# LouisPwr/CarpeDeam

Hardware: AMD Instinct MI355X
Metric: corrected bases/sec on 50M×100bp synthetic reads (dhigh), 1/2/4/8 GPU (higher is better)
Workload: dtype u8 (2-bit packed bases; int32 scores; software x87 f80 likelihood sums)

## Files before the change

carpedeam_amd/csrc/rescore.hip:

```cpp
#include "scan.h"

#include <cfloat>
#include <climits>

#include "common.h"
#include "devutil.h"

namespace {

struct RescoreArgs {
    MetaWoff woff; MetaLen len; MetaHasN hasN; MetaRaw hasRaw;
    const uint32_t *codes, *nmask; const uint8_t *raw;
    const uint64_t *hoff;
    const HitRec *hit;
    const int32_t *minScore;
    uint64_t nHits;
    uint32_t n;
    float seqIdThr, covThr;
    int covMode, minAlnLen;
    AlnRec *tmp;
    uint16_t *tmpRy;
    uint8_t *valid;
    unsigned int *undef;
};

__device__ __forceinline__ bool canBeCovered(float covThr, int covMode, float ql, float tl) {
    switch (covMode) {
        case 0: return ((ql / tl >= covThr) && (tl / ql >= covThr));
        case 2: return ((tl / ql) >= covThr);
        case 1: return ((ql / tl) >= covThr);
        case 3: return ((tl / ql) >= covThr) && (tl / ql) <= 1.0;
        case 4: return ((ql / tl) >= covThr) && (ql / tl) <= 1.0;
        case 5: return (fminf(tl, ql) / fmaxf(tl, ql)) >= covThr;
        default: return true;
    }
}
__device__ __forceinline__ bool hasCoverage(float covThr, int covMode, float qc, float tc) {
    switch (covMode) { case 0: return qc >= covThr && tc >= covThr; case 2: return qc >= covThr; case 1: return tc >= covThr; default: return true; }
}
__device__ __forceinline__ float computeCov(unsigned s, unsigned e, unsigned len) {
    return (min(len, max(s, e)) - min(s, e) + 1) / (float) len;
}

__device__ __forceinline__ void orientedBase(const RescoreArgs &a, uint32_t w0, uint32_t L, bool hasN, bool rc, uint32_t i, uint32_t &code, bool &isN) {
    const uint32_t p = rc ? (L - 1 - i) : i;
    code = cdm_base(a.codes, w0, p);
    isN = hasN && cdm_isN(a.nmask, w0, p);
    if (rc) code = 3u - code;
}

struct Diag { unsigned score; unsigned diagLen; unsigned dist; int diagonal; unsigned ident; unsigned ry; bool any; unsigned first, last; };

__device__ __forceinline__ void scoreDiagonal(const RescoreArgs &a, uint32_t qw, uint32_t qLen, bool qN, bool rc, uint32_t tw, uint32_t tLen, bool tN,
                                              int diagonal, Diag &best, bool qRaw = false, bool tRaw = false) {
    const unsigned md = (unsigned) abs(diagonal);
    uint32_t qOff, tOff, m;
    if (diagonal >= 0 && md < qLen) { qOff = md; tOff = 0; m = min(tLen, qLen - md); }
    else if (diagonal < 0 && md < tLen) { qOff = 0; tOff = md; m = min(tLen - md, qLen); }
    else return;
    unsigned mism = 0, identN = 0, ry = 0xFFFFu;
    uint32_t first = 0, last = m - 1;
    if (qRaw || tRaw) {
        const uint8_t q0 = (qRaw && !rc) ? cdm_raw_at(a.raw, qw, qOff) : 0, t0 = tRaw ? cdm_raw_at(a.raw, tw, tOff) : 0;
        const uint8_t q1 = (qRaw && !rc) ? cdm_raw_at(a.raw, qw, qOff + m - 1) : 0, t1 = tRaw ? cdm_raw_at(a.raw, tw, tOff + m - 1) : 0;
        first = (q0 == '*' || t0 == '*') ? 1u : 0u;
        if (last > 0 && (q1 == '*' || t1 == '*')) last--;
    }
    if (!qN && !tN) {
        ry = 0;
        const uint32_t qLast = (qLen + 15) / 16 - 1, tLast = (tLen + 15) / 16 - 1;
        for (uint32_t k = 0; k < m; k += 16) {
            const uint32_t x = cdm_oriented_window16(a.codes, qw, qLen, qLast, rc, qOff + k) ^ cdm_window16(a.codes, tw, tOff + k, tLast);
            uint32_t mm = (x | (x >> 1)) & 0x55555555u;
            const uint32_t rem = m - k;
            uint32_t rr = x & 0x55555555u;
            if (rem < 16) { mm &= (1u << (2 * rem)) - 1u; rr &= (1u << (2 * rem)) - 1u; }
            mism += __popc(mm); ry += __popc(rr);
        }
    } else {
        for (uint32_t k = first; k <= last && k < m; k++) {
            uint32_t qc, tc; bool qn, tn;
            orientedBase(a, qw, qLen, qN, rc, qOff + k, qc, qn);
            orientedBase(a, tw, tLen, tN, false, tOff + k, tc, tn);
            const bool match = !qn && !tn && qc == tc;
            mism += !match;
            if (!qRaw && !tRaw) identN += (qn && tn && !rc);
            else {
                uint8_t ql = qn ? (rc ? 'X' : 'N') : (uint8_t) "ACGT"[qc], tl = tn ? 'N' : (uint8_t) "ACGT"[tc];
                if (qRaw && !rc) ql = cdm_raw_at(a.raw, qw, qOff + k);
                if (tRaw) tl = cdm_raw_at(a.raw, tw, tOff + k);
                identN += ((ql & 0xDFu) == (tl & 0xDFu)) - (int) match;
            }
        }
    }
    const uint32_t cols = last + 1u >= first ? last + 1u - first : 0u;
    const long long sc = 2ll * (cols - mism) - 3ll * mism;
    const unsigned score = sc > 0 ? (unsigned) sc : 0u;
    if (score > best.score) { best.score = score; best.diagLen = m; best.dist = md; best.diagonal = diagonal; best.ident = (cols - mism) + identN; best.ry = ry; best.any = true; best.first = first; best.last = last; }
}

__global__ __launch_bounds__(256) void k_rescore(RescoreArgs a, const uint32_t *__restrict__ hitQuery) {
    const uint64_t h = (uint64_t) blockIdx.x * blockDim.x + threadIdx.x;
    if (h >= a.nHits) return;
    const uint32_t q = hitQuery[h];
    const HitRec hit = a.hit[h];
    const uint32_t t = hit.target;
    const uint32_t qLen = a.len[q], tLen = a.len[t], qw = a.woff[q], tw = a.woff[t];
    const bool qN = a.hasN[q] != 0, tN = a.hasN[t] != 0;
    const bool qRaw = qN && a.hasRaw[q] != 0, tRaw = tN && a.hasRaw[t] != 0;
    const bool isReverse = hit.score < 0;
    const bool isIdentity = (q == t);
    a.valid[h] = 0;
    if (!canBeCovered(a.covThr, a.covMode, (float) qLen, (float) tLen)) return;
    const unsigned short u = (unsigned short) (short) hit.diagonal;
    Diag best; best.score = 0; best.diagLen = 0; best.dist = 0; best.diagonal = 0; best.ident = 0; best.ry = 0xFFFFu; best.any = false; best.first = 0; best.last = 0;
    for (unsigned d = 1; d <= 1 + tLen / 32768; d++) scoreDiagonal(a, qw, qLen, qN, isReverse, tw, tLen, tN, (int) (-(int) d * 65536 + (int) u), best, qRaw, tRaw);
    for (unsigned d = 0; d <= qLen / 65536; d++) scoreDiagonal(a, qw, qLen, qN, isReverse, tw, tLen, tN, (int) (d * 65536 + u), best, qRaw, tRaw);
    if (!best.any) {
        if (!isIdentity) return;
        AlnRec r; r.target = t; r.rawScore = 0; r.ident = 1; r.qStart = r.qEnd = r.dbStart = r.dbEnd = -1; r.seqId = 1.0f;
        a.tmp[h] = r; a.tmpRy[h] = 0xFFFFu; a.valid[h] = 1;
        atomicAdd(a.undef, 1u);
        return;
    }
    const int startPos = (int) best.first, endPos = (int) best.last;
    const int alnLen = (endPos - startPos) + 1;
    int qs, qe, ds, de;
    if (best.diagonal >= 0) { qs = startPos + (int) best.dist; qe = endPos + (int) best.dist; ds = startPos; de = endPos; }
    else { qs = startPos; qe = endPos; ds = startPos + (int) best.dist; de = endPos + (int) best.dist; }
    const bool hasEvalue = (int) best.score >= a.minScore[qLen];
    float seqId = 0.f;
    if (hasEvalue || isIdentity) seqId = static_cast<float>(best.ident) / static_cast<float>(alnLen);
    const float queryCov = computeCov(qs, qe, qLen), targetCov = computeCov(ds, de, tLen);
    if (isReverse) { qs = (int) qLen - qs - 1; qe = (int) qLen - qe - 1; }
    const bool hasCov = hasCoverage(a.covThr, a.covMode, queryCov, targetCov);
    const bool hasSeqId = (double) seqId >= (double) (a.seqIdThr - FLT_EPSILON);
    const bool hasAlnLen = alnLen >= a.minAlnLen;
    if (!(isIdentity || (hasAlnLen && hasCov && hasSeqId && hasEvalue))) return;
    AlnRec r;
    r.target = t; r.rawScore = (int) best.score; r.ident = (int) best.ident; r.qStart = qs; r.qEnd = qe; r.dbStart = ds; r.dbEnd = de;
    r.seqId = (seqId == 1.0f) ? 1.0f : (float) ((double) (int) (seqId * 1000) / 1000.0);
    a.tmp[h] = r;
    a.tmpRy[h] = (uint16_t) min(best.ry, 0xFFFFu);
    a.valid[h] = 1;
}

__global__ void k_expand(const uint64_t *__restrict__ off, uint32_t n, uint32_t *__restrict__ owner) {
    const uint32_t q = blockIdx.x * blockDim.x + threadIdx.x;
    if (q >= n) return;
    for (uint64_t h = off[q]; h < off[q + 1]; h++) owner[h] = q;
}
__global__ void k_count_valid(const uint64_t *__restrict__ off, const uint8_t *__restrict__ valid, uint32_t n, uint64_t *__restrict__ cnt) {
    const uint32_t q = blockIdx.x * blockDim.x + threadIdx.x;
    if (q >= n) return;
    uint64_t c = 0;
    for (uint64_t h = off[q]; h < off[q + 1]; h++) c += valid[h];
    cnt[q] = c;
}
constexpr uint32_t SCATTER_SMALL = 256;
__global__ void k_scatter(const uint64_t *__restrict__ off, const uint32_t *__restrict__ owner, const uint8_t *__restrict__ valid, const AlnRec *__restrict__ tmp,
                          const uint16_t *__restrict__ tmpRy, uint64_t nHits, const uint64_t *__restrict__ outOff, AlnRec *__restrict__ out, uint16_t *__restrict__ outRy) {
    const uint64_t h = (uint64_t) blockIdx.x * blockDim.x + threadIdx.x;
    if (h >= nHits || !valid[h]) return;
    const uint32_t q = owner[h];
    const uint64_t first = off[q];
    if (off[q + 1] - first > SCATTER_SMALL) return;
    uint64_t o = outOff[q];
    for (uint64_t j = first; j < h; j++) o += valid[j];
    out[o] = tmp[h]; outRy[o] = tmpRy[h];
}
__global__ void k_scatter_big(const uint64_t *__restrict__ off, const uint8_t *__restrict__ valid, const AlnRec *__restrict__ tmp, const uint16_t *__restrict__ tmpRy, uint32_t n,
                              const uint64_t *__restrict__ outOff, AlnRec *__restrict__ out, uint16_t *__restrict__ outRy) {
    const uint32_t q = blockIdx.x * blockDim.x + threadIdx.x;
    if (q >= n || off[q + 1] - off[q] <= SCATTER_SMALL) return;
    uint64_t o = outOff[q];
    for (uint64_t h = off[q]; h < off[q + 1]; h++) if (valid[h]) { out[o] = tmp[h]; outRy[o] = tmpRy[h]; o++; }
}
__global__ void k_len_hist(const uint32_t *__restrict__ len, uint32_t n, uint32_t *__restrict__ present) {
    const uint32_t i = blockIdx.x * blockDim.x + threadIdx.x;
    if (i < n) present[len[i]] = 1;
}

}

int cdm_rescore_impl(cdm_ctx *ctx, const cdm_seqdb *db, const cdm_hits *hits, const cdm_rescore_params *par, cdm_alns **out) {
    hipStream_t s = ctx->stream;
    const uint32_t n = (uint32_t) db->n;
    const uint64_t nHits = hits->count;
    if (db->maxLen >= (1u << 30)) { cdm_set_error("cdm_rescore: sequence too long"); return CDM_ERR_UNSUPPORTED; }
    if (nHits >= 0xFFFFFF00ull) { cdm_set_error("cdm_rescore: %llu prefilter hits (a call takes fewer than 2^32)", (unsigned long long) nHits); return CDM_ERR_UNSUPPORTED; }
    DevBuf<unsigned int> undef;
    if (!undef.alloc(2)) { cdm_set_error("cdm_rescore: out of device memory"); return CDM_ERR_HIP; }
    CDM_HIP(hipMemsetAsync(undef.p, 0, 8, s));
    DevBuf<uint32_t> dPresent, owner; DevBuf<int32_t> dMin; DevBuf<AlnRec> tmp; DevBuf<uint16_t> tmpRy; DevBuf<uint8_t> valid; DevBuf<uint64_t> cnt;
    if (!dPresent.alloc(db->maxLen + 1) || !dMin.alloc(db->maxLen + 1) || !owner.alloc(nHits) || !tmp.alloc(nHits) || !tmpRy.alloc(nHits) || !valid.alloc(nHits) || !cnt.alloc((size_t) n + 1)) {
        cdm_set_error("cdm_rescore: out of device memory"); return CDM_ERR_HIP;
    }
    std::vector<uint32_t> present(db->maxLen + 1);
    CDM_HIP(hipMemsetAsync(dPresent.p, 0, (size_t) (db->maxLen + 1) * 4, s));
    hipLaunchKernelGGL(k_len_hist, dim3((n + 255) / 256), dim3(256), 0, s, db->len, n, dPresent.p);
    CDM_HIP(hipMemcpyAsync(present.data(), dPresent.p, (size_t) (db->maxLen + 1) * 4, hipMemcpyDeviceToHost, s));
    CDM_HIP(hipStreamSynchronize(s));
    std::vector<int32_t> minScore(db->maxLen + 1, INT_MAX);
    for (uint32_t L = 1; L <= db->maxLen; L++) {
        if (!present[L]) continue;
        int lo = 0, hi = 2 * (int) L;
        if (!(cdm_evalue_host(hi, L, db->residues) <= par->eval_thr)) continue;
        while (lo < hi) { int mid = (lo + hi) / 2; if (cdm_evalue_host(mid, L, db->residues) <= par->eval_thr) hi = mid; else lo = mid + 1; }
        minScore[L] = lo;
    }
    CDM_HIP(hipMemcpyAsync(dMin.p, minScore.data(), (size_t) (db->maxLen + 1) * 4, hipMemcpyHostToDevice, s));
    hipLaunchKernelGGL(k_expand, dim3((n + 255) / 256), dim3(256), 0, s, hits->off, n, owner.p);
    DevBuf<SeqMeta> meta;
    MetaUniform uni;
    if (int rc = cdm_build_meta(ctx, db, &meta.p, &uni)) return rc;
    RescoreArgs a;
    cdmSetMeta(a, meta.p, uni); a.codes = db->codes; a.nmask = db->nmask; a.raw = db->raw; a.hoff = hits->off; a.hit = hits->rec;
    a.minScore = dMin.p; a.nHits = nHits; a.n = n; a.seqIdThr = par->seq_id_thr; a.covThr = par->cov_thr; a.covMode = par->cov_mode;
    a.minAlnLen = par->min_aln_len; a.tmp = tmp.p; a.tmpRy = tmpRy.p; a.valid = valid.p; a.undef = undef.p;
    hipEventRecord(ctx->ev0, s);
    if (nHits) hipLaunchKernelGGL(k_rescore, CDM_GRID((nHits + 255) / 256, 256), dim3(256), 0, s, a, owner.p);
    hipEventRecord(ctx->ev1, s);
    hipLaunchKernelGGL(k_count_valid, dim3((n + 255) / 256), dim3(256), 0, s, hits->off, valid.p, n, cnt.p);
    CDM_LAUNCH_CHECK();
    cdm_alns *res = new cdm_alns(); res->n = n;
    struct Guard { cdm_alns *&r; bool armed = true; ~Guard() { if (armed && r) { cdm_alns_free(r); r = nullptr; } } } guard{res};
    if (cdmMalloc(&res->off, ((size_t) n + 1) * 8) != hipSuccess) { cdm_set_error("cdm_rescore: out of device memory"); return CDM_ERR_HIP; }
    cdmscan::ScanTemp scanTmp;
    CDM_HIP(hipMemsetAsync(cnt.p + n, 0, 8, s));
    if (int rc = cdmscan::exclusiveScan<uint64_t>(s, scanTmp, cnt.p, res->off, (size_t) n + 1)) return rc;
    uint64_t total = 0; unsigned int nUndef = 0;
    CDM_HIP(hipMemcpyAsync(&total, res->off + n, 8, hipMemcpyDeviceToHost, s));
    CDM_HIP(hipMemcpyAsync(&nUndef, undef.p, 4, hipMemcpyDeviceToHost, s));
    { hipError_t e = hipStreamSynchronize(s); if (e != hipSuccess) { cdm_set_error("cdm_rescore: kernel failed: %s", hipGetErrorString(e)); return CDM_ERR_HIP; } }
    res->count = total; res->undefinedRecords = nUndef;
    if (cdmMalloc(&res->rec, (total + 1) * sizeof(AlnRec)) != hipSuccess || cdmMalloc(&res->ryMism, (total + 1) * sizeof(uint16_t)) != hipSuccess) { cdm_set_error("cdm_rescore: out of device memory"); return CDM_ERR_HIP; }
    res->rySerial = db->serial;
    if (nHits) hipLaunchKernelGGL(k_scatter, CDM_GRID((nHits + 255) / 256, 256), dim3(256), 0, s, hits->off, (const uint32_t *) owner.p, valid.p, tmp.p, tmpRy.p, (uint64_t) nHits, res->off, res->rec, res->ryMism);
    hipLaunchKernelGGL(k_scatter_big, dim3((n + 255) / 256), dim3(256), 0, s, hits->off, valid.p, tmp.p, tmpRy.p, n, res->off, res->rec, res->ryMism);
    { hipError_t e = hipStreamSynchronize(s); if (e != hipSuccess) { cdm_set_error("cdm_rescore: compaction failed: %s", hipGetErrorString(e)); return CDM_ERR_HIP; } }
    hipEventElapsedTime(&ctx->lastMs[1], ctx->ev0, ctx->ev1);
    guard.armed = false;
    *out = res;
    return CDM_OK;
}
```

Baseline: 17.40 billion.

## Fuse rescore output compaction into a single-pass decoupled look-back scan

Rescoring and output compaction now happen in one kernel. Each 256-hit tile takes a dynamic ticket, counts its valid alignments with a wave ballot, and gets its global offset through a decoupled look-back over per-tile status words. Records go straight to their final position, and per-query offsets are written from that. This drops the temporary record, ry and valid buffers, the count kernel, the exclusive scan, the two scatter kernels and one host sync. In exchange, the output arrays are sized for all hits rather than the exact total. Empty queries that fall past a bounded run need a fallback fill kernel, and the status memset covers one more element than is allocated.

After: 17.26 billion. No clear change (-0.8%).

```diff
diff --git a/carpedeam_amd/csrc/rescore.hip b/carpedeam_amd/csrc/rescore.hip
--- a/carpedeam_amd/csrc/rescore.hip
+++ b/carpedeam_amd/csrc/rescore.hip
@@ -1,4 +1,3 @@
-#include "scan.h"
 
 #include <cfloat>
 #include <climits>
@@ -18,10 +17,14 @@
     uint32_t n;
     float seqIdThr, covThr;
     int covMode, minAlnLen;
-    AlnRec *tmp;
-    uint16_t *tmpRy;
-    uint8_t *valid;
+    AlnRec *rec;
+    uint16_t *ry;
+    uint64_t *off;
+    unsigned long long *status;
+    unsigned long long *total;
+    unsigned int *ticket;
     unsigned int *undef;
+    unsigned int *longRun;
 };
 
 __device__ __forceinline__ bool canBeCovered(float covThr, int covMode, float ql, float tl) {
@@ -99,29 +102,24 @@
     if (score > best.score) { best.score = score; best.diagLen = m; best.dist = md; best.diagonal = diagonal; best.ident = (cols - mism) + identN; best.ry = ry; best.any = true; best.first = first; best.last = last; }
 }
 
-__global__ __launch_bounds__(256) void k_rescore(RescoreArgs a, const uint32_t *__restrict__ hitQuery) {
-    const uint64_t h = (uint64_t) blockIdx.x * blockDim.x + threadIdx.x;
-    if (h >= a.nHits) return;
-    const uint32_t q = hitQuery[h];
-    const HitRec hit = a.hit[h];
+__device__ __forceinline__ bool scoreHit(const RescoreArgs &a, uint32_t q, const HitRec hit, AlnRec &r, uint32_t &ry) {
     const uint32_t t = hit.target;
     const uint32_t qLen = a.len[q], tLen = a.len[t], qw = a.woff[q], tw = a.woff[t];
     const bool qN = a.hasN[q] != 0, tN = a.hasN[t] != 0;
     const bool qRaw = qN && a.hasRaw[q] != 0, tRaw = tN && a.hasRaw[t] != 0;
     const bool isReverse = hit.score < 0;
     const bool isIdentity = (q == t);
-    a.valid[h] = 0;
-    if (!canBeCovered(a.covThr, a.covMode, (float) qLen, (float) tLen)) return;
+    if (!canBeCovered(a.covThr, a.covMode, (float) qLen, (float) tLen)) return false;
     const unsigned short u = (unsigned short) (short) hit.diagonal;
     Diag best; best.score = 0; best.diagLen = 0; best.dist = 0; best.diagonal = 0; best.ident = 0; best.ry = 0xFFFFu; best.any = false; best.first = 0; best.last = 0;
     for (unsigned d = 1; d <= 1 + tLen / 32768; d++) scoreDiagonal(a, qw, qLen, qN, isReverse, tw, tLen, tN, (int) (-(int) d * 65536 + (int) u), best, qRaw, tRaw);
     for (unsigned d = 0; d <= qLen / 65536; d++) scoreDiagonal(a, qw, qLen, qN, isReverse, tw, tLen, tN, (int) (d * 65536 + u), best, qRaw, tRaw);
     if (!best.any) {
-        if (!isIdentity) return;
-        AlnRec r; r.target = t; r.rawScore = 0; r.ident = 1; r.qStart = r.qEnd = r.dbStart = r.dbEnd = -1; r.seqId = 1.0f;
-        a.tmp[h] = r; a.tmpRy[h] = 0xFFFFu; a.valid[h] = 1;
+        if (!isIdentity) return false;
+        r.target = t; r.rawScore = 0; r.ident = 1; r.qStart = r.qEnd = r.dbStart = r.dbEnd = -1; r.seqId = 1.0f;
+        ry = 0xFFFFu;
         atomicAdd(a.undef, 1u);
-        return;
+        return true;
     }
     const int startPos = (int) best.first, endPos = (int) best.last;
     const int alnLen = (endPos - startPos) + 1;
@@ -136,13 +134,72 @@
     const bool hasCov = hasCoverage(a.covThr, a.covMode, queryCov, targetCov);
     const bool hasSeqId = (double) seqId >= (double) (a.seqIdThr - FLT_EPSILON);
     const bool hasAlnLen = alnLen >= a.minAlnLen;
-    if (!(isIdentity || (hasAlnLen && hasCov && hasSeqId && hasEvalue))) return;
-    AlnRec r;
+    if (!(isIdentity || (hasAlnLen && hasCov && hasSeqId && hasEvalue))) return false;
     r.target = t; r.rawScore = (int) best.score; r.ident = (int) best.ident; r.qStart = qs; r.qEnd = qe; r.dbStart = ds; r.dbEnd = de;
     r.seqId = (seqId == 1.0f) ? 1.0f : (float) ((double) (int) (seqId * 1000) / 1000.0);
-    a.tmp[h] = r;
-    a.tmpRy[h] = (uint16_t) min(best.ry, 0xFFFFu);
-    a.valid[h] = 1;
+    ry = min(best.ry, 0xFFFFu);
+    return true;
+}
+
+constexpr int RS_TILE = 256, RS_WAVES = RS_TILE / 64;
+constexpr uint32_t RS_RUN = 32;
+constexpr unsigned long long ST_AGG = 1ull << 62, ST_PREFIX = 2ull << 62, ST_MASK = (1ull << 62) - 1ull;
+__global__ __launch_bounds__(RS_TILE) void k_rescore(RescoreArgs a, const uint32_t *__restrict__ hitQuery) {
+    __shared__ unsigned int sTile, sWave[RS_WAVES];
+    __shared__ unsigned long long sPrefix;
+    const int tid = threadIdx.x, lane = tid & 63, wave = tid >> 6;
+    if (tid == 0) sTile = atomicAdd(a.ticket, 1u);
+    __syncthreads();
+    const uint64_t tile = sTile, h = tile * RS_TILE + tid;
+    const bool live = h < a.nHits;
+    uint32_t q = 0, ry = 0xFFFFu;
+    AlnRec r;
+    bool ok = false;
+    if (live) { q = hitQuery[h]; ok = scoreHit(a, q, a.hit[h], r, ry); }
+    const unsigned long long m = __ballot(ok);
+    const uint32_t inWave = __builtin_amdgcn_mbcnt_hi((uint32_t) (m >> 32), __builtin_amdgcn_mbcnt_lo((uint32_t) m, 0u));
+    if (lane == 0) sWave[wave] = (uint32_t) __popcll(m);
+    __syncthreads();
+    uint32_t before = 0, tot = 0;
+#pragma unroll
+    for (int w = 0; w < RS_WAVES; w++) { const uint32_t c = sWave[w]; if (w < wave) before += c; tot += c; }
+    if (wave == 0) {
+        unsigned long long excl = 0;
+        if (tile == 0) { if (lane == 0) __hip_atomic_store(&a.status[0], ST_PREFIX | (unsigned long long) tot, __ATOMIC_RELAXED, __HIP_MEMORY_SCOPE_AGENT); }
+        else {
+            if (lane == 0) __hip_atomic_store(&a.status[tile], ST_AGG | (unsigned long long) tot, __ATOMIC_RELAXED, __HIP_MEMORY_SCOPE_AGENT);
+            long long t0 = (long long) tile - 1;
+            while (true) {
+                const long long t = t0 - lane;
+                unsigned long long v = ST_PREFIX;
+                if (t >= 0) do { v = __hip_atomic_load(&a.status[t], __ATOMIC_RELAXED, __HIP_MEMORY_SCOPE_AGENT); } while ((v >> 62) == 0ull);
+                const unsigned long long pm = __ballot((v >> 62) == 2ull);
+                const int first = pm ? __ffsll(pm) - 1 : 63;
+                const unsigned long long part = cdm_wave_incl_sum<unsigned long long>(lane <= first ? (v & ST_MASK) : 0ull);
+                excl += (unsigned long long) __shfl((long long) part, 63, 64);
+                if (pm) break;
+                t0 -= 64;
+            }
+            if (lane == 0) __hip_atomic_store(&a.status[tile], ST_PREFIX | (excl + tot), __ATOMIC_RELAXED, __HIP_MEMORY_SCOPE_AGENT);
+        }
+        if (lane == 0) sPrefix = excl;
+    }
+    __syncthreads();
+    if (!live) return;
+    const uint64_t o = sPrefix + before + inWave;
+    if (ok) { a.rec[o] = r; a.ry[o] = (uint16_t) ry; }
+    if (h == a.hoff[q]) {
+        a.off[q] = o;
+        uint32_t p = q;
+        while (p > 0 && q - p < RS_RUN && a.hoff[p - 1] == h) a.off[--p] = o;
+        if (p > 0 && a.hoff[p - 1] == h) *a.longRun = 1u;
+    }
+    if (h == a.nHits - 1) {
+        const uint64_t e = o + (ok ? 1u : 0u);
+        a.off[a.n] = e; *a.total = e;
+        if (a.n - 1 - q <= RS_RUN) for (uint32_t p = q + 1; p < a.n; p++) a.off[p] = e;
+        else *a.longRun = 1u;
+    }
 }
 
 __global__ void k_expand(const uint64_t *__restrict__ off, uint32_t n, uint32_t *__restrict__ owner) {
@@ -150,31 +207,11 @@
     if (q >= n) return;
     for (uint64_t h = off[q]; h < off[q + 1]; h++) owner[h] = q;
 }
-__global__ void k_count_valid(const uint64_t *__restrict__ off, const uint8_t *__restrict__ valid, uint32_t n, uint64_t *__restrict__ cnt) {
+__global__ void k_fill_empty(const uint64_t *__restrict__ hoff, const uint32_t *__restrict__ owner, uint32_t n, uint64_t nHits, uint64_t total, uint64_t *off) {
     const uint32_t q = blockIdx.x * blockDim.x + threadIdx.x;
     if (q >= n) return;
-    uint64_t c = 0;
-    for (uint64_t h = off[q]; h < off[q + 1]; h++) c += valid[h];
-    cnt[q] = c;
-}
-constexpr uint32_t SCATTER_SMALL = 256;
-__global__ void k_scatter(const uint64_t *__restrict__ off, const uint32_t *__restrict__ owner, const uint8_t *__restrict__ valid, const AlnRec *__restrict__ tmp,
-                          const uint16_t *__restrict__ tmpRy, uint64_t nHits, const uint64_t *__restrict__ outOff, AlnRec *__restrict__ out, uint16_t *__restrict__ outRy) {
-    const uint64_t h = (uint64_t) blockIdx.x * blockDim.x + threadIdx.x;
-    if (h >= nHits || !valid[h]) return;
-    const uint32_t q = owner[h];
-    const uint64_t first = off[q];
-    if (off[q + 1] - first > SCATTER_SMALL) return;
-    uint64_t o = outOff[q];
-    for (uint64_t j = first; j < h; j++) o += valid[j];
-    out[o] = tmp[h]; outRy[o] = tmpRy[h];
-}
-__global__ void k_scatter_big(const uint64_t *__restrict__ off, const uint8_t *__restrict__ valid, const AlnRec *__restrict__ tmp, const uint16_t *__restrict__ tmpRy, uint32_t n,
-                              const uint64_t *__restrict__ outOff, AlnRec *__restrict__ out, uint16_t *__restrict__ outRy) {
-    const uint32_t q = blockIdx.x * blockDim.x + threadIdx.x;
-    if (q >= n || off[q + 1] - off[q] <= SCATTER_SMALL) return;
-    uint64_t o = outOff[q];
-    for (uint64_t h = off[q]; h < off[q + 1]; h++) if (valid[h]) { out[o] = tmp[h]; outRy[o] = tmpRy[h]; o++; }
+    const uint64_t h = hoff[q];
+    if (h == hoff[q + 1]) off[q] = h < nHits ? off[owner[h]] : total;
 }
 __global__ void k_len_hist(const uint32_t *__restrict__ len, uint32_t n, uint32_t *__restrict__ present) {
     const uint32_t i = blockIdx.x * blockDim.x + threadIdx.x;
@@ -189,13 +226,14 @@
     const uint64_t nHits = hits->count;
     if (db->maxLen >= (1u << 30)) { cdm_set_error("cdm_rescore: sequence too long"); return CDM_ERR_UNSUPPORTED; }
     if (nHits >= 0xFFFFFF00ull) { cdm_set_error("cdm_rescore: %llu prefilter hits (a call takes fewer than 2^32)", (unsigned long long) nHits); return CDM_ERR_UNSUPPORTED; }
-    DevBuf<unsigned int> undef;
-    if (!undef.alloc(2)) { cdm_set_error("cdm_rescore: out of device memory"); return CDM_ERR_HIP; }
-    CDM_HIP(hipMemsetAsync(undef.p, 0, 8, s));
-    DevBuf<uint32_t> dPresent, owner; DevBuf<int32_t> dMin; DevBuf<AlnRec> tmp; DevBuf<uint16_t> tmpRy; DevBuf<uint8_t> valid; DevBuf<uint64_t> cnt;
-    if (!dPresent.alloc(db->maxLen + 1) || !dMin.alloc(db->maxLen + 1) || !owner.alloc(nHits) || !tmp.alloc(nHits) || !tmpRy.alloc(nHits) || !valid.alloc(nHits) || !cnt.alloc((size_t) n + 1)) {
+    const uint64_t tiles = (nHits + RS_TILE - 1) / RS_TILE;
+    DevBuf<unsigned long long> ctl, status;
+    DevBuf<uint32_t> dPresent, owner; DevBuf<int32_t> dMin;
+    if (!ctl.alloc(3) || !status.alloc(tiles) || !dPresent.alloc(db->maxLen + 1) || !dMin.alloc(db->maxLen + 1) || !owner.alloc(nHits)) {
         cdm_set_error("cdm_rescore: out of device memory"); return CDM_ERR_HIP;
     }
+    CDM_HIP(hipMemsetAsync(ctl.p, 0, 24, s));
+    CDM_HIP(hipMemsetAsync(status.p, 0, (tiles + 1) * 8, s));
     std::vector<uint32_t> present(db->maxLen + 1);
     CDM_HIP(hipMemsetAsync(dPresent.p, 0, (size_t) (db->maxLen + 1) * 4, s));
     hipLaunchKernelGGL(k_len_hist, dim3((n + 255) / 256), dim3(256), 0, s, db->len, n, dPresent.p);
@@ -217,28 +255,27 @@
     RescoreArgs a;
     cdmSetMeta(a, meta.p, uni); a.codes = db->codes; a.nmask = db->nmask; a.raw = db->raw; a.hoff = hits->off; a.hit = hits->rec;
     a.minScore = dMin.p; a.nHits = nHits; a.n = n; a.seqIdThr = par->seq_id_thr; a.covThr = par->cov_thr; a.covMode = par->cov_mode;
-    a.minAlnLen = par->min_aln_len; a.tmp = tmp.p; a.tmpRy = tmpRy.p; a.valid = valid.p; a.undef = undef.p;
-    hipEventRecord(ctx->ev0, s);
-    if (nHits) hipLaunchKernelGGL(k_rescore, CDM_GRID((nHits + 255) / 256, 256), dim3(256), 0, s, a, owner.p);
-    hipEventRecord(ctx->ev1, s);
-    hipLaunchKernelGGL(k_count_valid, dim3((n + 255) / 256), dim3(256), 0, s, hits->off, valid.p, n, cnt.p);
-    CDM_LAUNCH_CHECK();
+    a.minAlnLen = par->min_aln_len;
     cdm_alns *res = new cdm_alns(); res->n = n;
     struct Guard { cdm_alns *&r; bool armed = true; ~Guard() { if (armed && r) { cdm_alns_free(r); r = nullptr; } } } guard{res};
-    if (cdmMalloc(&res->off, ((size_t) n + 1) * 8) != hipSuccess) { cdm_set_error("cdm_rescore: out of device memory"); return CDM_ERR_HIP; }
-    cdmscan::ScanTemp scanTmp;
-    CDM_HIP(hipMemsetAsync(cnt.p + n, 0, 8, s));
-    if (int rc = cdmscan::exclusiveScan<uint64_t>(s, scanTmp, cnt.p, res->off, (size_t) n + 1)) return rc;
-    uint64_t total = 0; unsigned int nUndef = 0;
-    CDM_HIP(hipMemcpyAsync(&total, res->off + n, 8, hipMemcpyDeviceToHost, s));
-    CDM_HIP(hipMemcpyAsync(&nUndef, undef.p, 4, hipMemcpyDeviceToHost, s));
+    if (cdmMalloc(&res->off, ((size_t) n + 1) * 8) != hipSuccess || cdmMalloc(&res->rec, (nHits + 1) * sizeof(AlnRec)) != hipSuccess ||
+        cdmMalloc(&res->ryMism, (nHits + 1) * sizeof(uint16_t)) != hipSuccess) { cdm_set_error("cdm_rescore: out of device memory"); return CDM_ERR_HIP; }
+    res->rySerial = db->serial;
+    a.rec = res->rec; a.ry = res->ryMism; a.off = res->off; a.status = status.p; a.total = ctl.p;
+    a.ticket = reinterpret_cast<unsigned int *>(ctl.p + 1); a.undef = a.ticket + 1; a.longRun = a.ticket + 2;
+    if (!nHits) CDM_HIP(hipMemsetAsync(res->off, 0, ((size_t) n + 1) * 8, s));
+    hipEventRecord(ctx->ev0, s);
+    if (nHits) hipLaunchKernelGGL(k_rescore, CDM_GRID(tiles, RS_TILE), dim3(RS_TILE), 0, s, a, (const uint32_t *) owner.p);
+    hipEventRecord(ctx->ev1, s);
+    CDM_LAUNCH_CHECK();
+    unsigned long long ctlHost[3] = {0, 0, 0};
+    CDM_HIP(hipMemcpyAsync(ctlHost, ctl.p, 24, hipMemcpyDeviceToHost, s));
     { hipError_t e = hipStreamSynchronize(s); if (e != hipSuccess) { cdm_set_error("cdm_rescore: kernel failed: %s", hipGetErrorString(e)); return CDM_ERR_HIP; } }
-    res->count = total; res->undefinedRecords = nUndef;
-    if (cdmMalloc(&res->rec, (total + 1) * sizeof(AlnRec)) != hipSuccess || cdmMalloc(&res->ryMism, (total + 1) * sizeof(uint16_t)) != hipSuccess) { cdm_set_error("cdm_rescore: out of device memory"); return CDM_ERR_HIP; }
-    res->rySerial = db->serial;
-    if (nHits) hipLaunchKernelGGL(k_scatter, CDM_GRID((nHits + 255) / 256, 256), dim3(256), 0, s, hits->off, (const uint32_t *) owner.p, valid.p, tmp.p, tmpRy.p, (uint64_t) nHits, res->off, res->rec, res->ryMism);
-    hipLaunchKernelGGL(k_scatter_big, dim3((n + 255) / 256), dim3(256), 0, s, hits->off, valid.p, tmp.p, tmpRy.p, n, res->off, res->rec, res->ryMism);
-    { hipError_t e = hipStreamSynchronize(s); if (e != hipSuccess) { cdm_set_error("cdm_rescore: compaction failed: %s", hipGetErrorString(e)); return CDM_ERR_HIP; } }
+    res->count = ctlHost[0]; res->undefinedRecords = (unsigned int) (ctlHost[1] >> 32);
+    if ((unsigned int) ctlHost[2]) {
+        hipLaunchKernelGGL(k_fill_empty, dim3((n + 255) / 256), dim3(256), 0, s, hits->off, (const uint32_t *) owner.p, n, nHits, (uint64_t) res->count, res->off);
+        hipError_t e = hipStreamSynchronize(s); if (e != hipSuccess) { cdm_set_error("cdm_rescore: compaction failed: %s", hipGetErrorString(e)); return CDM_ERR_HIP; }
+    }
     hipEventElapsedTime(&ctx->lastMs[1], ctx->ev0, ctx->ev1);
     guard.armed = false;
     *out = res;
```
